# pranavkantgaur/3dscan

Hardware: AMD Instinct MI355X
Metric: Mpixels/s decode+unwrap+triangulate @1920×1080 (higher is better)
Workload: dtype f64

## Files before the change

### 3dscan_amd/csrc/sl3d_capi_context.cpp

```cpp
#include "sl3d_capi_internal.h"

static thread_local std::string g_create_err;

int sl3d_fail(sl3d_ctx *c, int code, const std::string &msg)
{
    if (c) c->err = msg;
    else g_create_err = msg;
    return code;
}

int sl3d_caught(sl3d_ctx *c, std::string *other) noexcept
{
    int code = SL3D_E_INTERNAL;
    const char *what = "unknown C++ exception";
    char buf[256];
    try {
        throw;
    } catch (const std::bad_alloc &) {
        code = SL3D_E_NOMEM;
        what = "out of host memory (std::bad_alloc)";
    } catch (const std::exception &e) {
        snprintf(buf, sizeof buf, "internal error: %s", e.what());
        what = buf;
    } catch (...) {
    }
    try {
        if (other) *other = what;
        else if (c) c->err = what;
        else g_create_err = what;
    } catch (...) {
    }
    return code;
}

extern "C" const char *sl3d_version(void) { return SL3D_VERSION_STRING " (gfx950, hip)"; }

extern "C" const char *sl3d_strerror(int s)
{
    switch (s) {
    case SL3D_OK: return "ok";
    case SL3D_E_INVALID_ARG: return "invalid argument";
    case SL3D_E_NO_DEVICE: return "no HIP device available (this library has no CPU fallback)";
    case SL3D_E_HIP: return "HIP runtime error";
    case SL3D_E_STATE: return "call order violated";
    case SL3D_E_UNSUPPORTED: return "unsupported configuration";
    case SL3D_E_NOMEM: return "out of memory";
    case SL3D_E_INTERNAL: return "internal error (a C++ exception was stopped at the C boundary)";
    default: return "unknown status";
    }
}

extern "C" const char *sl3d_last_error(const sl3d_ctx *ctx) { return ctx ? ctx->err.c_str() : g_create_err.c_str(); }

// ... 116 lines not shown
    x->quad_blocks = mask_prepare_blocks(P);
    CREATE_CHK(hipHostMalloc((void **)&x->h_quad_part, V * (size_t)x->quad_blocks * sizeof(unsigned long long), hipHostMallocMapped));
    memset((void *)x->h_quad_part, 0, V * (size_t)x->quad_blocks * sizeof(unsigned long long));
    CREATE_CHK(hipHostGetDevicePointer((void **)&x->d_quad_part, (void *)x->h_quad_part, 0));
    x->quad_seq.assign(V, 0u);
    x->quad_sum_seq.assign(V, 0u);
    x->quad_sum.assign(V, 0u);
    x->quad_last.assign(V, ~0u);
    x->quad_src.resize(V);
    for (size_t v = 0; v < V; v++) x->quad_src[v] = (int)v;
    x->quad_kind.assign(V, 0);
    x->pend.assign(V, sl3d_ctx::PendingMask());
    x->eager_mask = (c.flags & SL3D_FLAG_EAGER_MASK) != 0;
    if (!x->keep && P.F == 3) {
        x->mi_part_stride = fused_maskin_part_stride(P);
        x->mi_part_words = fused_maskin_part_words(P);
        CREATE_CHK(hipHostMalloc((void **)&x->h_mi_part, V * (size_t)x->mi_part_stride * sizeof(unsigned), hipHostMallocMapped));
        memset((void *)x->h_mi_part, 0, V * (size_t)x->mi_part_stride * sizeof(unsigned));
        CREATE_CHK(hipHostGetDevicePointer((void **)&x->d_mi_part, (void *)x->h_mi_part, 0));
    }
    CREATE_CHK(hipMemsetAsync(x->d_mask, 0, V * P.mask_view_stride, x->stream));
    CREATE_CHK(hipMemsetAsync(x->d_frames, 0, V * P.view_stride, x->stream));
    CREATE_CHK(hipMemsetAsync(x->d_valid, 0, V * P.px_view_stride, x->stream));
    CREATE_CHK(hipMemsetAsync(x->d_points, 0, V * P.px_view_stride * 3 * sizeof(float), x->stream));
    CREATE_CHK(hipMemsetAsync(x->d_band, 0, V * P.px_view_stride, x->stream));
    P.frames = x->d_frames; P.mask = x->d_mask; P.points = x->d_points; P.valid = x->d_valid; P.band = x->d_band;
    {
        static std::mutex mu;
        static std::set<int> verified;
        std::lock_guard<std::mutex> lk(mu);
        if (!verified.count(c.device)) {
            std::vector<float> tab;
            build_atan_tables(tab);
            const size_t n = (size_t)SL3D_ATAN_T1 * SL3D_ATAN_T2;
            float *d_tab = nullptr;
            unsigned *d_cnt = nullptr, h_cnt = 0;
            CREATE_CHK(hipMalloc((void **)&d_tab, 2 * n * sizeof(float)));
            CREATE_CHK(hipMalloc((void **)&d_cnt, sizeof(unsigned)));
            CREATE_CHK(hipMemcpyAsync(d_tab, tab.data(), 2 * n * sizeof(float), hipMemcpyHostToDevice, x->stream));
            CREATE_CHK(hipMemsetAsync(d_cnt, 0, sizeof(unsigned), x->stream));
            CREATE_CHK((hipError_t)launch_atan_selfcheck(d_tab, d_tab + n, d_cnt, x->stream));
            CREATE_CHK(hipMemcpyAsync(&h_cnt, d_cnt, sizeof(unsigned), hipMemcpyDeviceToHost, x->stream));
            CREATE_CHK(hipStreamSynchronize(x->stream));
            (void)hipFree(d_tab);
            (void)hipFree(d_cnt);
            if (h_cnt != 0) {
                g_create_err = "device atan2 differs from the host libm atan2 on " + std::to_string(h_cnt) +
                               " of 521731 lattice points: bit-exact parity cannot be guaranteed on this host/GPU pair";
                        return SL3D_E_UNSUPPORTED;
            }
            verified.insert(c.device);
        }
    }
    if (x->keep) {
        const size_t n = V * P.px_view_stride;
        for (int a = 0; a < 2; a++) {
            ALLOC(P.wrapped[a], n); ALLOC(P.unwrapped[a], n); ALLOC(P.code[a], n);
            ALLOC(P.valid_axis[a], n); ALLOC(P.dbg3[a], n); ALLOC(P.dbg4[a], n);
            CREATE_CHK(hipMemsetAsync(P.wrapped[a], 0, n * 4, x->stream));
            CREATE_CHK(hipMemsetAsync(P.unwrapped[a], 0, n * 4, x->stream));
            CREATE_CHK(hipMemsetAsync(P.code[a], 0xff, n * 4, x->stream));
            CREATE_CHK(hipMemsetAsync(P.valid_axis[a], 0, n, x->stream));
            CREATE_CHK(hipMemsetAsync(P.dbg3[a], 0, n, x->stream));
            CREATE_CHK(hipMemsetAsync(P.dbg4[a], 0, n, x->stream));
        }
        ALLOC(P.cpmap, n * 2); ALLOC(P.ipoints, n * 3);
        CREATE_CHK(hipMemsetAsync(P.cpmap, 0, n * 16, x->stream));
        CREATE_CHK(hipMemsetAsync(P.ipoints, 0, n * 24, x->stream));
    }
#if defined(SL3D_MEASURE) && defined(SL3D_TRACE)
    {
        const size_t blocks = ((((size_t)(P.pitch >> 2) * P.H + 255) / 256) + 7) & ~(size_t)7;
        x->dbg_words = V * blocks * 4 * 8;
        ALLOC(P.dbg, x->dbg_words);
        CREATE_CHK(hipMemsetAsync(P.dbg, 0, x->dbg_words * sizeof(unsigned long long), x->stream));
    }
#endif
    CREATE_CHK(hipStreamSynchronize(x->stream));
#undef ALLOC
#undef CREATE_CHK
    unwind.p = nullptr;
    *out = x;
    return SL3D_OK;
}
SL3D_CATCH(nullptr)

extern "C" void sl3d_destroy(sl3d_ctx *x)
try {
    if (!x) return;
    DeviceGuard dev_guard_(x->cfg.device);
    for (int l = 0; l < 2; l++)
        if (x->lane[l]) (void)hipStreamSynchronize(x->lane[l]);
    if (x->stream) (void)hipStreamSynchronize(x->stream);
    for (int l = 0; l < 2; l++) {
        if (x->ev_lane[l]) (void)hipEventDestroy(x->ev_lane[l]);
        if (x->lane[l]) (void)hipStreamDestroy(x->lane[l]);
    }
    if (x->ev_main) (void)hipEventDestroy(x->ev_main);
    for (void *p : x->allocs) (void)hipFree(p);
    if (x->h_counts) (void)hipHostFree(x->h_counts);
    if (x->h_quad_part) (void)hipHostFree((void *)x->h_quad_part);
    if (x->h_mi_part) (void)hipHostFree((void *)x->h_mi_part);
    for (hipEvent_t e : x->ev_up) (void)hipEventDestroy(e);
    for (hipEvent_t e : x->ev_done) (void)hipEventDestroy(e);
    for (hipEvent_t e : x->ev_down) (void)hipEventDestroy(e);
    if (x->s_h2d) (void)hipStreamDestroy(x->s_h2d);
// ... 160 lines not shown
```

### 3dscan_amd/csrc/sl3d_ctx.h

```cpp
#pragma once
#include <hip/hip_runtime.h>

#include <string>
#include <vector>

#include "../../include/sl3d.h"
#include "sl3d_internal.h"
#include "sl3d_lanes.h"

using namespace sl3d;

struct sl3d_ctx {
    sl3d_config cfg{};
    KParams P{};
    DevCal C{};
    SynthParams S{};
    bool have_cal = false;
    int rig = 0;
    bool keep = false;
    bool own_stream = false;
    hipStream_t stream = nullptr;
    hipEvent_t ev0 = nullptr, ev1 = nullptr;
    bool lanes_ok = false;
    hipStream_t lane[2] = {nullptr, nullptr};
// ... 8 lines not shown
    volatile unsigned long long *h_quad_part = nullptr;
    unsigned long long *d_quad_part = nullptr;
    int quad_blocks = 0;
    std::vector<unsigned> quad_seq;
    std::vector<int> quad_src;
    mutable std::vector<unsigned> quad_sum_seq, quad_sum;
    mutable std::vector<unsigned> quad_last;
    unsigned mask_seq = 0;
    struct PendingMask {
        bool pending = false;
        bool ours = false;
        uintptr_t origin = 0;
        size_t stride = 0;
        int lo = 0, hi = 0;
    };
    std::vector<PendingMask> pend;
    int n_pending = 0;
    bool eager_mask = false;
    volatile unsigned *h_mi_part = nullptr;
    unsigned *d_mi_part = nullptr;
    unsigned mi_part_stride = 0, mi_part_words = 0;
    std::vector<uint8_t> quad_kind;
    struct { int n_views = 0, cmode = 0; bool keep = false, prefer_gated = false, maskin = false; } last_fused;
    float *d_points = nullptr;
    unsigned *d_blk_cnt = nullptr;
    unsigned long long *d_blk_off = nullptr;
    unsigned long long *d_total = nullptr;
    float *d_cloud = nullptr;
    float *d_reg = nullptr;
    uint8_t *d_raw = nullptr;
    bool raw_map_valid = false;
    double Kc_raw[9] = {0}, dc_raw[5] = {0};
    uint8_t *d_und = nullptr;
    size_t und_bytes = 0;
    double und_key[16] = {0};
    bool und_map_valid = false;
    hipStream_t s_h2d = nullptr, s_d2h = nullptr;
    std::vector<hipEvent_t> ev_up, ev_done, ev_down;
    float *d_clouds = nullptr;
    unsigned *d_blk_cnt_all = nullptr;
    unsigned long long *d_blk_off_all = nullptr, *d_totals = nullptr;
    unsigned *d_seg_counts = nullptr;
    unsigned long long *d_seg_offsets = nullptr;
    float *d_packed = nullptr;
    std::vector<uint8_t> scan_state;
    bool clouds_ready = false;
    unsigned long long *h_counts = nullptr;
    uint8_t *d_texture = nullptr;
    uint8_t *d_cloud_rgb = nullptr;
    std::vector<char> have_texture;
    double *d_cam_tab = nullptr;
    size_t cam_tab_doubles = 0;
    float2 *d_proj_disp = nullptr;
    RadEntry *d_proj_rad = nullptr;
    uint8_t *d_pattern = nullptr, *d_profile = nullptr;
    size_t pattern_pitch = 0;
    uint8_t *d_colrow = nullptr;
    size_t colrow_bytes = 0;
    DevCal *d_cal = nullptr;
    size_t mask_rows = 0;
    size_t dbg_words = 0;
};

__attribute__((visibility("hidden"))) int sl3d_fail(sl3d_ctx *c, int code, const std::string &msg);
#define fail sl3d_fail
__attribute__((visibility("hidden"))) int sl3d_caught(sl3d_ctx *c, std::string *err_of_other_owner = nullptr) noexcept;
#define SL3D_CATCH(ctx) catch (...) { return sl3d_caught(ctx); }
#define SL3D_CATCH_RETURN(value) catch (...) { (void)sl3d_caught(nullptr); return value; }
#define SL3D_CATCH_VOID catch (...) { (void)sl3d_caught(nullptr); }
__attribute__((visibility("hidden"))) int sl3d_process_views_enqueue(sl3d_ctx *x, int n_views, const uint8_t *const *planes, size_t stride, float *xyz,
                                                                     size_t xyz_view_stride, uint8_t *valid, size_t valid_view_stride, size_t out_width);
__attribute__((visibility("hidden"))) int sl3d_process_views_wait(sl3d_ctx *x);

#define HIPCHK(c, call)                                                                             \
    do {                                                                                            \
        hipError_t e_ = (call);                                                                     \
        if (e_ != hipSuccess)                                                                       \
            return fail((c), SL3D_E_HIP, std::string(#call) + ": " + hipGetErrorString(e_));        \
    } while (0)

#define HIPCHK_DRAIN(c, call)                                                                       \
    do {                                                                                            \
        hipError_t e_ = (call);                                                                     \
        if (e_ != hipSuccess) {                                                                     \
            (void)hipStreamSynchronize((c)->stream);                                                \
            return fail((c), SL3D_E_HIP, std::string(#call) + ": " + hipGetErrorString(e_));        \
        }                                                                                           \
    } while (0)

struct DeviceGuard {
    int prev = -1, dev;
    hipError_t err = hipSuccess;
    explicit DeviceGuard(int d) : dev(d)
    {
        if (hipGetDevice(&prev) != hipSuccess) prev = -1;
        if (prev != dev) err = hipSetDevice(dev);
    }
    ~DeviceGuard()
    {
        if (prev >= 0 && prev != dev) (void)hipSetDevice(prev);
    }
    DeviceGuard(const DeviceGuard &) = delete;
    DeviceGuard &operator=(const DeviceGuard &) = delete;
};
#define ON_DEVICE_QUIET(x)                 \
    DeviceGuard dev_guard_((x)->cfg.device); \
// ... 10 lines not shown
```

### 3dscan_amd/csrc/sl3d_fused.h

```cpp
#pragma once
#include <stddef.h>
#include <stdlib.h>
#include "sl3d_device.h"
#include "sl3d_maskbits.h"

#define SL3D_BLOCK 256
#define SL3D_OCC 4
#define SL3D_SMALL_BLOCK SL3D_BLOCK

#if !defined(SL3D_MEASURE) || !defined(SL3D_ABLATE)
#undef SL3D_ABLATE
#define SL3D_ABLATE 0
#endif
#if defined(SL3D_MEASURE) && defined(SL3D_TRACE)
#define SL3D_STAMP(k)                                                                                                               \
    do {                                                                                                                            \
           \
        if ((CMODE & 2) == 0 && !KEEP && P.dbg)                                                                                           \
            P.dbg[(((size_t)blockIdx.y * gridDim.x + blockIdx.x) * 4 + (threadIdx.x >> 6)) * 8 + (k)] = wall_clock64();              \
    } while (0)
#else
#define SL3D_STAMP(k)
#endif
#ifdef SL3D_MEASURE
#define SL3D_ABLATE_RT(P) ((P).ablate)
#else
#define SL3D_ABLATE_RT(P) 0
#endif

namespace sl3d {


struct PixelResult {
    float x, y, z;
    bool valid;
};

template <typename CalP>
__device__ __forceinline__ PixelResult parity_chain(const KParams &P, CalP Cp, const PinnedRows &PR, int gx, int gy, double cu, double cv, float wv,
                                                    float wh, int code_v, int code_h, size_t keep_off)
{
    PixelResult R;
    const float nanv = __builtin_nanf("");
    R.x = R.y = R.z = nanv;
    const bool in_v = gx >= 1 && gx <= P.fullW - 2;
    const bool in_h = gy >= 1 && gy <= P.fullH - 2;
    const float uvv = unwrap_value(wv, code_v), uhv = unwrap_value(wh, code_h);
    const float uv = in_v ? uvv : 0.0f;
    const float uh = in_h ? uhv : 0.0f;
    long cx, cy;
    double cxd, cyd;
    const bool okx = correspond(uv, P.fwv, P.PW, cx, cxd);
    const bool oky = correspond(uh, P.fwh, P.PH, cy, cyd);
    R.valid = okx && oky;
    P.wrapped[0][keep_off] = wv;
    P.wrapped[1][keep_off] = wh;
    P.unwrapped[0][keep_off] = uv;
    P.unwrapped[1][keep_off] = uh;
    P.code[0][keep_off] = code_v;
    P.code[1][keep_off] = code_h;
    P.cpmap[2 * keep_off + 0] = R.valid ? cx : 0;
    P.cpmap[2 * keep_off + 1] = R.valid ? cy : 0;
    if (R.valid) {
        double up, vp, X[3];
        const auto &C = *Cp;
        if (C.proj.identity) {
            up = cxd;
            vp = cyd;
        } else {
            undistort_reproject(cxd, cyd, C.proj, up, vp);
        }
        triangulate_px(C, PR, cu, cv, up, vp, X);
        R.x = (float)X[0];
        R.y = (float)X[1];
        R.z = (float)X[2];
        P.ipoints[3 * keep_off + 0] = X[0];
        P.ipoints[3 * keep_off + 1] = X[1];
        P.ipoints[3 * keep_off + 2] = X[2];
    }
    return R;
}

__device__ __forceinline__ bool correspond_px(const KParams &P, int gx, int gy, float wv, float wh, int code_v, int code_h, int &cx, int &cy)
{
    const bool in_v = gx >= 1 && gx <= P.fullW - 2;
    const bool in_h = gy >= 1 && gy <= P.fullH - 2;
    float uvv = unwrap_value(wv, code_v), uhv = unwrap_value(wh, code_h);
    asm volatile("" : "+v"(uvv));
    asm volatile("" : "+v"(uhv));
    float uv = in_v ? uvv : 0.0f;
    float uh = in_h ? uhv : 0.0f;
    asm volatile("" : "+v"(uv));
    asm volatile("" : "+v"(uh));
    long lx, ly;
    double dxd, dyd;
    const bool okx = correspond(uv, P.fwv, P.PW, lx, dxd);
    const bool oky = correspond(uh, P.fwh, P.PH, ly, dyd);
    cx = (int)lx;
    cy = (int)ly;
    return okx && oky;
}

template <int RIG, typename CalP>
__device__ __forceinline__ void triangulate_from(const KParams &P, CalP Cp, const PinnedRows &PR, double cu, double cv, int cx, int cy, float2 d, bool table,
                                                 const RadEntry *s_rad, float &x, float &y, float &z)
{
    const auto &C = *Cp;
    const double cxd = (double)cx, cyd = (double)cy;
    double X[3];
    bool singular = false;
    if (RIG == 3) {
        const double dx = cxd - C.proj.cx, dy = cyd - C.proj.cy;
        const double x0 = dx * C.proj.ifx, y0 = dy * C.proj.ify;
        const double s = radial_lookup(s_rad, P.proj_rad_scale, fma(x0, x0, y0 * y0));
        triangulate_camframe(C, PR, cu, cv, fma(dx, s, cxd), fma(dy, s, cyd), X, singular);
    } else if (RIG == 1) {
        triangulate_camframe(C, PR, cu, cv, cxd, cyd, X, singular);
    } else if (RIG == 2) {
        triangulate_camframe(C, PR, cu, cv, cxd + (double)d.x, cyd + (double)d.y, X, singular);
    } else {
        double up = cxd, vp = cyd;
        if (table) {
            up = cxd + (double)d.x;
            vp = cyd + (double)d.y;
        } else if (!C.proj.identity) {
            undistort_reproject(cxd, cyd, C.proj, up, vp);
        }
        triangulate_px(C, PR, cu, cv, up, vp, X);
    }
    x = (float)X[0];
    y = (float)X[1];
    z = (float)X[2];
    if (RIG != 0 && singular) x = y = z = 0.0f;
}

struct Item {
    unsigned tile;
    int cq, row;
    int gx0, gy;
    int v_begin, v_end;
    bool alive;
    unsigned lane_off;
};

template <bool KIND2 = true>
__device__ __forceinline__ void cam_table_request(const KParams &P, const Item &it, double (&t)[8])
{
    const size_t i0 = (size_t)it.row * P.pitch + (size_t)it.cq * 4;
    if (!KIND2 || P.use_cam_table == 1) {
        const double2 *tp = (const double2 *)(P.cam_tab + i0);
        const double2 a = tp[0], b = tp[1];
        t[0] = a.x; t[1] = a.y; t[2] = b.x; t[3] = b.y;
    } else {
        const double2 *tp = (const double2 *)(P.cam_tab + 2 * i0);
        const double2 a = tp[0], b = tp[1], c = tp[2], d = tp[3];
// ... 282 lines not shown
            if (PLANES == 1 || i < N) {
                g[a][i] = ldg32(vb + (size_t)(pg + (unsigned)i * psv), lo);
                iv[a][i] = ldg32(vb + (size_t)(pg + (unsigned)(N + i) * psv), lo);
            }
        }
    }
}

template <int NMAX, int PLANES>
__device__ __forceinline__ void decode_gray(const unsigned (&g)[2][NMAX], const unsigned (&iv)[2][NMAX], int Nv, int Nh, unsigned (&code)[2][2])
{
#pragma unroll
    for (int a = 0; a < 2; a++) {
        const int N = a == 0 ? Nv : Nh;
        const unsigned H = 0x80808080u;
        unsigned bacc = 0;
        unsigned hi = 0, lo = 0;
        if (PLANES >= 2) {
            int pad = NMAX - N;
            if (PLANES == 3) pad = __builtin_amdgcn_readfirstlane(pad);
            asm volatile("" : "+s"(pad));
#pragma unroll
            for (int i = 0; i < NMAX; i++) {
                const unsigned x = g[a][i], y = iv[a][i];
                const unsigned t = (x | H) - (y & ~H);
                const unsigned ge = __builtin_amdgcn_bitop3_b32(x, y, t, 0xB2);
                const unsigned Hm = i >= pad ? H : 0u;
                bacc = __builtin_amdgcn_bitop3_b32(bacc, ge, Hm, 0x78);
                if (i < NMAX - 8) hi = (hi << 1) | (bacc >> 7);
                else lo = (lo << 1) | (bacc >> 7);
            }
            code[a][0] = __builtin_amdgcn_perm(hi, lo, 0x05010400u);
            code[a][1] = __builtin_amdgcn_perm(hi, lo, 0x07030602u);
            continue;
        }
#pragma unroll
        for (int i = 0; i < NMAX; i++) {
            if (i < N) {
                const unsigned x = g[a][i], y = iv[a][i];
                const unsigned t = (x | H) - (y & ~H);
                const unsigned ge = __builtin_amdgcn_bitop3_b32(x, y, t, 0xB2);
                bacc = __builtin_amdgcn_bitop3_b32(bacc, ge, H, 0x78);
                if (i < N - 8) hi = (hi << 1) | (bacc >> 7);
                else lo = (lo << 1) | (bacc >> 7);
            }
        }
        code[a][0] = __builtin_amdgcn_perm(hi, lo, 0x05010400u);
        code[a][1] = __builtin_amdgcn_perm(hi, lo, 0x07030602u);
    }
}

template <bool RCP_TAB>
__device__ __forceinline__ unsigned pixel_A(const KParams &P, const Item &it, int F, int i, int k, unsigned vbits, const unsigned (&f)[2][4],
                                            const unsigned (&code)[2][2], const double *s_rcp, int *pair_cp)
{
    const int sh = 8 * i;
    const int code_v = (int)((code[0][0] >> (16 * i)) & 0xffffu);
    const int code_h = (int)((code[1][0] >> (16 * i)) & 0xffffu);
    const AtanK AK = atan_consts<true>();
    float wv = wrapped_phase<RCP_TAB>(F, (f[0][0] >> sh) & 255, (f[0][1] >> sh) & 255, (f[0][2] >> sh) & 255, (f[0][3] >> sh) & 255, s_rcp, AK);
    float wh = wrapped_phase<RCP_TAB>(F, (f[1][0] >> sh) & 255, (f[1][1] >> sh) & 255, (f[1][2] >> sh) & 255, (f[1][3] >> sh) & 255, s_rcp, AK);
    wv = shift_pi(wv);
    wh = shift_pi(wh);
    int cx, cy;
    const bool ok = correspond_px(P, it.gx0 + k, it.gy, wv, wh, code_v, code_h, cx, cy) && ((vbits >> i) & 1u);
    pair_cp[3 * i] = ok ? cx : 0;
    pair_cp[3 * i + 1] = ok ? cy : 0;
    return ok ? 1u : 0u;
}

template <bool RCP_TAB>
__device__ __forceinline__ void phase_A_pair(const KParams &P, const Item &it, int F, int j, unsigned &vbits, unsigned (&f)[2][4], unsigned (&code)[2][2],
                                             const double *s_rcp, int *pair_cp, unsigned &vout)
{
    const unsigned ok0 = pixel_A<RCP_TAB>(P, it, F, 0, 2 * j, vbits, f, code, s_rcp, pair_cp), ok1 = pixel_A<RCP_TAB>(P, it, F, 1, 2 * j + 1, vbits, f, code, s_rcp, pair_cp);
    vout = (vout >> 16) | (ok0 << 16) | (ok1 << 24);
#pragma unroll
    for (int a = 0; a < 2; a++) {
#pragma unroll
        for (int p = 0; p < 4; p++) f[a][p] >>= 16;
        code[a][0] = code[a][1];
    }
    vbits >>= 2;
}

template <bool RCP_TAB, bool UNROLL>
__device__ __forceinline__ unsigned phase_A(const KParams &P, const Item &it, int F, unsigned vbits, unsigned (&f)[2][4], unsigned (&code)[2][2],
                                            const double *s_rcp, int *my_cp)
{
    unsigned vout = 0;
#pragma unroll(UNROLL ? 2 : 1)
    for (int j = 0; j < 2; j++) {
        int j8 = j * 8;
        if (!UNROLL) asm volatile("" : "+v"(j8));
        phase_A_pair<RCP_TAB>(P, it, F, j, vbits, f, code, s_rcp, my_cp + (UNROLL ? 6 * j : ((j8 << 1) + j8) >> 2), vout);
    }
    return vout;
}

template <bool RCP_TAB>
__device__ __forceinline__ void wrapped_quad(int F, const unsigned (&f)[2][4], const double *s_rcp, float (&w)[2][4])
{
    const AtanK AK = atan_consts<true>();
#pragma unroll
    for (int k = 0; k < 4; k++) {
        const int sh = 8 * k;
#pragma unroll
        for (int a = 0; a < 2; a++)
            w[a][k] = shift_pi(wrapped_phase<RCP_TAB>(F, (f[a][0] >> sh) & 255, (f[a][1] >> sh) & 255, (f[a][2] >> sh) & 255, (f[a][3] >> sh) & 255, s_rcp, AK));
    }
}

__device__ __forceinline__ unsigned correspond_quad(const KParams &P, const Item &it, unsigned vbits, const float (&w)[2][4], const unsigned (&code)[2][2], int *my_cp)
{
    unsigned vout = 0;
#pragma unroll
    for (int k = 0; k < 4; k++) {
        const int code_v = (int)((code[0][k >> 1] >> (16 * (k & 1))) & 0xffffu);
        const int code_h = (int)((code[1][k >> 1] >> (16 * (k & 1))) & 0xffffu);
        int cx, cy;
        const bool ok = correspond_px(P, it.gx0 + k, it.gy, w[0][k], w[1][k], code_v, code_h, cx, cy) && ((vbits >> k) & 1u);
        my_cp[3 * k] = ok ? cx : 0;
        my_cp[3 * k + 1] = ok ? cy : 0;
        vout |= (ok ? 1u : 0u) << (8 * k);
    }
    return vout;
}

__device__ __forceinline__ void gather_B(const KParams &P, bool proj_table, const int *my_cp, float2 (&d)[4])
{
#pragma unroll
    for (int k = 0; k < 4; k++) d[k] = make_float2(0.f, 0.f);
    if (proj_table) {
        const GLOBAL_AS uint8_t *tab = opaque((const uint8_t *)P.proj_disp);
        const unsigned pw = (unsigned)P.PW;
#pragma unroll
        for (int k = 0; k < 4; k++) d[k] = ldg_f2(tab, ((unsigned)my_cp[3 * k + 1] * pw + (unsigned)my_cp[3 * k]) * 8u);
    }
}

template <int RIG, bool UNROLL>
__device__ __forceinline__ void phase_B(const KParams &P, const DevCal *Cglobal, const PinnedRows &PR, bool proj_table, unsigned vout, float2 (&d)[4],
                                        const double *my_cam, const int *my_cp, float *my_xyz, const RadEntry *s_rad)
{
    const float nanv = __builtin_nanf("");
    unsigned vb = vout;
#pragma unroll(UNROLL ? 2 : 1)
    for (int j = 0; j < 2; j++) {
        int j8 = j * 8;
        if (!UNROLL) asm volatile("" : "+v"(j8));
        const int pair_words = UNROLL ? 6 * j : ((j8 << 1) + j8) >> 2;
        const int *cp = my_cp + pair_words;
        float *xyz = my_xyz + pair_words;
        const double *cam = my_cam + (UNROLL ? 4 * j : j8 >> 1);
#pragma unroll
        for (int i = 0; i < 2; i++) {
            float x, y, z;
            triangulate_from<RIG>(P, opaque_const(Cglobal), PR, cam[2 * i], cam[2 * i + 1], cp[3 * i], cp[3 * i + 1], d[i], proj_table, s_rad, x, y, z);
            const bool ok = ((vb >> (8 * i)) & 1u) != 0u;
            xyz[3 * i + 0] = ok ? x : nanv;
            xyz[3 * i + 1] = ok ? y : nanv;
            xyz[3 * i + 2] = ok ? z : nanv;
        }
        d[0] = d[2];
        d[1] = d[3];
        vb >>= 16;
    }
}

template <bool RCP_TAB>
__device__ __forceinline__ unsigned parity_pixels(const KParams &P, const DevCal *Cglobal, const PinnedRows &PR, const Item &it, int F, unsigned vbits,
                                                  const unsigned (&f)[2][4], const unsigned (&code)[2][2], const double *s_rcp, const double *my_cam,
                                                  float *my_xyz, size_t px)
{
// ... 109 lines not shown
            if ((vout >> (8 * k)) & 1u) {
                wbase[3 * rank + 0] = q[3 * k + 0];
                wbase[3 * rank + 1] = q[3 * k + 1];
                wbase[3 * rank + 2] = q[3 * k + 2];
                rank++;
            }
    }
    wave_lds_handoff();
    const unsigned chunks = (3u * total + 3u) >> 2;
    typedef float f32x4 __attribute__((ext_vector_type(4)));
    const f32x4 *wb4 = (const f32x4 *)wbase;
    GLOBAL_AS uint8_t *out = opaque_out(slot);
#pragma unroll
    for (int c3 = 0; c3 < 3; c3++) {
        const unsigned i = (unsigned)c3 * 64u + lane_;
        if (i < chunks) stg_nt(out, lane_ * 16u + (unsigned)c3 * 1024u, wb4[i]);
    }
    wave_lds_handoff();
}

template <bool KEEP, bool FGEN, bool SEG>
__device__ __forceinline__ unsigned valid_bits(const Item &it, int F, const MaskQuad &m)
{
    if (SEG && !it.alive) return 0u;
    return (FGEN && F == 5) ? 0u : (!KEEP && (SL3D_ABLATE & 2)) ? 0xfu : mask_quad_bits(m);
}

template <int RIG>
struct RadialLds {
    __device__ __forceinline__ static RadEntry *get() { return nullptr; }
};
template <>
struct RadialLds<3> {
    __device__ __forceinline__ static RadEntry *get()
    {
        __shared__ RadEntry tab[SL3D_RAD_NODES];
        return tab;
    }
};

template <bool KEEP, int NMAX, bool FGEN, bool EXACT, int RIG, int CMODE, bool RCPT, bool EARLY_>
__global__ __launch_bounds__(RCPT ? SL3D_BLOCK : SL3D_SMALL_BLOCK, SL3D_OCC) void k_fused(const KParams P, const DevCal *__restrict__ Cglobal, int first_view, int n_views, int vpt)
{
    constexpr bool SEG = (CMODE & 2) != 0;
    constexpr bool MASKIN = (CMODE & 4) != 0;
    constexpr int BLK = RCPT ? SL3D_BLOCK : SL3D_SMALL_BLOCK;
    static_assert((CMODE & ~6) == 0, "0 = dense planes, 2 = segmented clouds (1 was round 2's look-back compaction), + 4 = MASKIN");
    static_assert(!MASKIN || (!KEEP && RIG != 0 && (RCPT ? !EARLY_ : EARLY_)),
                  "MASKIN: the pipelined small-launch instantiations, and the gated large-launch ones (views known to be sparsely selected)");
    static_assert(!(KEEP && CMODE != 0), "the parity mode writes dense planes");
    static_assert(!(KEEP && RIG != 0), "the parity mode evaluates everything with the reference's operation order");
    __shared__ __attribute__((aligned(16))) float s_xyz[BLK * 12];
    __shared__ __attribute__((aligned(16))) double s_cam[BLK * 8];
    __shared__ __attribute__((aligned(16))) double s_rcp[RCPT ? SL3D_RCP_TAB : 1];
    RadEntry *const s_rad = RadialLds<RIG>::get();
    static_assert(RIG != 3 || SL3D_BLOCK == SL3D_RAD_NODES, "one table node per thread");
    SL3D_STAMP(0);
    constexpr bool PIPE = !KEEP && RIG != 0;
    static_assert(RCPT || EARLY_ == PIPE, "the small-launch instantiation: early requests iff pipelined");
    constexpr bool EARLY = EARLY_ && PIPE;
    constexpr bool REQ_FIRST = PIPE;
    typedef unsigned u32x4 __attribute__((ext_vector_type(4)));
    u32x4 rad_node = {0u, 0u, 0u, 0u};
    if (RIG == 3) rad_node = ((const u32x4 *)P.proj_rad)[(blockIdx.x & 7u) * SL3D_RAD_STRIDE + threadIdx.x];
    if (!REQ_FIRST) {
        if (RIG == 3) ((u32x4 *)s_rad)[threadIdx.x] = rad_node;
        if (RCPT) fill_rcp_table(s_rcp);
        if (RCPT || RIG == 3) __syncthreads();
    }
    SL3D_STAMP(1);
    const int F = FGEN ? P.F : 3;
    float *my_xyz = s_xyz + threadIdx.x * 12;
    double *my_cam = s_cam + threadIdx.x * 8;
    int *my_cp = (int *)my_xyz;
    constexpr bool UNROLL = !RCPT;
#ifdef SL3D_NO_SPLIT
    constexpr bool SPLIT = false;
#else
    constexpr bool SPLIT = EARLY;
#endif

    constexpr int PLANES = EXACT ? 1 : (!KEEP && NMAX <= 12) ? ((MASKIN && RCPT) ? 3 : 2) : 0;
    const int Nv = EXACT ? NMAX : P.Nv, Nh = EXACT ? NMAX : P.Nh;
    const bool proj_table = RIG == 2 || (RIG == 0 && !KEEP && P.proj_disp != nullptr);

    Item it;
    MaskQuad mq;
    double camt[8] = {0, 0, 0, 0, 0, 0, 0, 0};
    unsigned mbits = 0u;
    mrow_t mw0 = {0u, 0u}, mw1 = mw0, mw2 = mw0, mw3 = mw0, mw4 = mw0;
    bool mfast = false;
    unsigned f[2][4], g[2][NMAX], iv[2][NMAX], code[2][2];
    if (!item_begin<RIG, SEG, REQ_FIRST, BLK, MASKIN>(P, Cglobal, blockIdx.x, (int)blockIdx.y, first_view, n_views, vpt, it, mq, camt, my_cam, mw0, mw1, mw2, mw3, mw4, mfast)) return;
    if (MASKIN) it.v_end = it.v_begin + 1;
    if (REQ_FIRST) {
        if (EARLY) {
            issue_fringe<FGEN>(P, it.v_begin, it.lane_off, F, Nv, f);
            issue_gray<NMAX, PLANES>(P, it.v_begin, it.lane_off, F, Nv, Nh, g, iv);
        }
        if (RCPT) fill_rcp_table(s_rcp);
        if (RIG == 3) ((u32x4 *)s_rad)[threadIdx.x] = rad_node;
        if (RCPT || RIG == 3) __syncthreads();
        if (!SEG && !it.alive) return;
        if (MASKIN) {
            if (it.alive) mbits = maskin_finish(P, it, it.v_begin, it.v_begin - first_view, mw0, mw1, mw2, mw3, mw4, mfast);
            maskin_count(P, it, it.v_begin, mbits);
        }
        if (P.use_cam_table) cam_table_finish<RIG, !MASKIN>(P, Cglobal, it, camt, my_cam);
    }
    SL3D_STAMP(2);
    unsigned vb_next = 0;
    if (PIPE) {
        vb_next = MASKIN ? (mbits & 0xfu) : valid_bits<KEEP, FGEN, SEG>(it, F, mq);
        if (!MASKIN && it.v_begin + 1 < it.v_end) mq = load_mask_quad(P, it.v_begin + 1, it.lane_off);
        if (!EARLY && vb_next != 0) {
            issue_fringe<FGEN>(P, it.v_begin, it.lane_off, F, Nv, f);
            issue_gray<NMAX, PLANES>(P, it.v_begin, it.lane_off, F, Nv, Nh, g, iv);
        }
    }
    const PinnedRows PR = pinned_rows<RIG>(Cglobal);
    constexpr bool DEFER = PIPE;
    unsigned pvout = 0;
    auto store_view = [&](int v, unsigned vo) {
        const size_t p = (size_t)v * P.px_view_stride + (size_t)it.lane_off;
        if (MASKIN && it.alive) maskin_store(P, it, v, mbits);
        if (SEG) store_segment(P, it, v, vo, s_xyz, my_xyz);
        else store_quad<KEEP>(P, s_xyz, my_xyz, p, vo);
    };
    for (int view = it.v_begin; view < it.v_end; view++) {
        unsigned vbits;
        if (PIPE) {
            vbits = vb_next;
        } else {
            vbits = valid_bits<KEEP, FGEN, SEG>(it, F, mq);
            if (view + 1 < it.v_end) mq = load_mask_quad(P, view + 1, it.lane_off);
        }
        const size_t px = (size_t)view * P.px_view_stride + (size_t)it.lane_off;
        unsigned vout = 0;
        if (KEEP) parity_init(P, px, vbits);
        if (!DEFER && !SEG && (KEEP || vbits == 0)) fill_nan(my_xyz);
        if (!PIPE && vbits != 0) {
            issue_fringe<FGEN>(P, view, it.lane_off, F, Nv, f);
            issue_gray<NMAX, PLANES>(P, view, it.lane_off, F, Nv, Nh, g, iv);
        }
        if (view == it.v_begin) SL3D_STAMP(3);
        float w[2][4];
        if (SPLIT && vbits != 0) {
            wrapped_quad<RCPT>(F, f, s_rcp, w);
            __builtin_amdgcn_sched_barrier(0);
        }
        if (vbits != 0) decode_gray<NMAX, PLANES>(g, iv, Nv, Nh, code);
        if (view == it.v_begin) SL3D_STAMP(4);
        unsigned vb_pre = 0;
        if (PIPE) {
            vb_pre = MASKIN ? 0u : valid_bits<KEEP, FGEN, SEG>(it, F, mq);
            asm volatile("" : "+v"(vb_pre));
        }
        if (DEFER) {
            if (view > it.v_begin) store_view(view - 1, pvout);
            if (!SEG && vbits == 0) fill_nan(my_xyz);
        }
        if (vbits != 0) {
            if (KEEP) vout = parity_pixels<RCPT>(P, Cglobal, PR, it, F, vbits, f, code, s_rcp, my_cam, my_xyz, px);
            else if (SPLIT) vout = correspond_quad(P, it, vbits, w, code, my_cp);
            else vout = phase_A<RCPT, UNROLL>(P, it, F, vbits, f, code, s_rcp, my_cp);
        }
        if (view == it.v_begin) SL3D_STAMP(5);
        if (PIPE && view + 1 < it.v_end) {
            vb_next = vb_pre;
            if (!MASKIN) mq = load_mask_quad(P, min(view + 2, it.v_end - 1), it.lane_off);
            if (vb_next != 0) {
                issue_fringe<FGEN>(P, view + 1, it.lane_off, F, Nv, f);
                issue_gray<NMAX, PLANES>(P, view + 1, it.lane_off, F, Nv, Nh, g, iv);
            }
        }
        if (!KEEP && vbits != 0) {
            float2 d[4];
            gather_B(P, proj_table, my_cp, d);
            phase_B<RIG, UNROLL>(P, Cglobal, PR, proj_table, vout, d, my_cam, my_cp, my_xyz, s_rad);
        }
        if (DEFER) {
            if (view == it.v_begin) SL3D_STAMP(6);
            pvout = vout;
            continue;
        }
        if (SEG) {
            store_segment(P, it, view, vout, s_xyz, my_xyz);
            continue;
        }
        if (view == it.v_begin) SL3D_STAMP(6);
        store_quad<KEEP>(P, s_xyz, my_xyz, px, vout);
        if (view == it.v_begin) SL3D_STAMP(7);
    }
    if (DEFER) {
        store_view(it.v_end - 1, pvout);
        SL3D_STAMP(7);
    }
}

struct FusedChoice {
    int nmax;
    bool exact, small;
    bool early;
};
inline FusedChoice choose_fused(bool keep, bool fgen, int cmode, int nv, int nh, int n_views, bool prefer_gated, int rig)
{
    FusedChoice c;
    const int m = nv > nh ? nv : nh;
    c.exact = !keep && !fgen && nv == nh && nv >= 6 && nv <= 12;
    if (c.exact) c.nmax = nv;
    else if (!keep && m <= 12 && nv > 0 && nh > 0) c.nmax = m < 6 ? 6 : m;
    else if (!keep) c.nmax = SL3D_MAX_GRAY;
    else c.nmax = m <= 8 ? 8 : (m <= 12 ? 12 : SL3D_MAX_GRAY);
    c.small = !keep && !fgen && n_views <= SL3D_SMALL_LAUNCH_VIEWS && !prefer_gated;
#ifdef SL3D_MEASURE
    if (getenv("SL3D_NO_SMALL")) c.small = false;
#endif
    const bool pipelined = !keep && rig != 0 && m <= 12 && nv > 0 && nh > 0;
// ... 112 lines not shown
```

### 3dscan_amd/csrc/sl3d_internal.h

```cpp
#pragma once
#include <stddef.h>
#include <stdint.h>

#include <hip/hip_vector_types.h>

#define SL3D_MASK_HALO 2
#define SL3D_MASK_LPAD 16
#define SL3D_ATAN_T1 511
#define SL3D_ATAN_T2 1021
#define SL3D_MAX_GRAY 16
#define SL3D_SEG_POINTS 256
#define SL3D_SMALL_LAUNCH_VIEWS 4

namespace sl3d {

struct Intr {
    double K[9];
    double ifx, ify, cx, cy;
    double k1, k2, p1, p2, k3;
    int has_dist;
    int affine;
    int has_tan;
    int plain;
    int identity;
// ... 37 lines not shown
    uintptr_t origin[SL3D_SMALL_LAUNCH_VIEWS];
    size_t stride;
    int bx0, bx1, r0, r1;
    int lo, hi;
    unsigned *part;
    unsigned part_stride;
    unsigned seq;
};

struct KParams {
    int W, H;
    int fullW, fullH;
    int col0, row0;
    int PW, PH;
    int F, Nv, Nh;
    int fwv, fwh;
    int ncodes_v, ncodes_h;
    int ablate;
    int pitch;
    int planes_per_view;
    size_t plane_stride;
    size_t view_stride;
    int mpitch;
    size_t mask_view_stride;
    const uint8_t *frames;
    const uint8_t *mask;
    const uint8_t *band;
    const float2 *proj_disp;
    const RadEntry *proj_rad;
    float proj_rad_scale;
    const double *cam_tab;
    int cam_tab_kind;
    int use_cam_table;
    float *points;
    uint8_t *valid;
    size_t px_view_stride;
    float *clouds;
    unsigned long long *cloud_totals;
    int n_tiles;
    int prefer_gated;
    unsigned *seg_counts;
    unsigned long long *seg_offsets;
    int n_segs;
    unsigned long long *dbg;
    float *wrapped[2];
    float *unwrapped[2];
    int32_t *code[2];
    uint8_t *valid_axis[2];
    uint8_t *dbg3[2];
    uint8_t *dbg4[2];
    int64_t *cpmap;
    double *ipoints;
    MaskIn mi;
};
static_assert(SL3D_SMALL_LAUNCH_VIEWS == 4, "KParams::mi_origin holds one entry per view of a small launch");

int launch_fused(const KParams &P, const DevCal *d_cal, int rig, int first_view, int n_views, bool keep, int cmode, void *stream, bool prefer_gated = false,
                 const MaskIn *mi = nullptr);
int fused_kernel_name(const KParams &P, int rig, int n_views, bool keep, int cmode, char *buf, size_t cap, bool prefer_gated = false, bool maskin = false);
bool fused_maskin_available(const KParams &P, int rig, int n_views, bool keep);
unsigned fused_maskin_part_stride(const KParams &P);
unsigned fused_maskin_part_words(const KParams &P);
int launch_seg_scan(const KParams &P, int first_view, int n_views, void *stream);
int launch_seg_close(const KParams &P, int first_view, int n_views, float *dst, size_t dst_view_stride_points, void *stream);
int launch_seg_close_scan(const KParams &P, int first_view, int n_views, float *dst, size_t dst_view_stride_points, unsigned long long capacity_points,
                          void *stream);
int launch_seg_register(const KParams &P, int view, float *out, const float R4[4], float tx, float ty, float tz, void *stream);
int fused_tiles(const KParams &P);
int launch_mask_prepare(const KParams &P, int first_view, int n_views, const MaskSrc &S, unsigned long long *partials, unsigned seq, void *stream);
int mask_prepare_blocks(const KParams &P);
int launch_to_colrow(const KParams &P, int view, int which, void *dst, void *stream);
int launch_mask_from_colrow(const KParams &P, const int *sel, int gx0, int gy0, int ncols, int nrows, uint8_t *raw, void *stream);
int launch_proj_table(const DevCal *d_cal, int PW, int PH, float2 *out, void *stream);
int launch_radial_table(const DevCal *d_cal, int which, double r2max, RadEntry *out, void *stream);
int launch_cam_table(const KParams &P, const DevCal *d_cal, int kind, double *out, void *stream);
int launch_wrap(const KParams &P, int view, int axis, void *stream);
int launch_unwrap(const KParams &P, int view, int axis, void *stream);
int launch_corr(const KParams &P, int view, void *stream);
int launch_tri(const KParams &P, const DevCal &C, int view, void *stream);
int launch_compact(const KParams &P, int view, unsigned *block_counts, unsigned long long *block_offsets, unsigned long long *total,
                   float *cloud, const uint8_t *texture, uint8_t *rgb_out, void *stream);
int launch_compact_views(const KParams &P, int first_view, int n_views, unsigned *block_counts, unsigned long long *block_offsets,
                         unsigned long long *totals, float *clouds, void *stream);
int launch_register(const float *in, float *out, long n, const float R4[4], float tx, float ty, float tz, void *stream);
int launch_synth(const KParams &P, const DevCal &C, const SynthParams &S, int view, void *stream);
int launch_undistort(const uint8_t *src, size_t sstride, uint8_t *dst, size_t dstride, int width, int height, int cn, const double K[9],
                     const double dist[5], short *m1, unsigned short *m2, bool build_map, void *stream);
int launch_undistort_planes(const uint8_t *src, size_t spitch, size_t splane, uint8_t *dst, size_t dpitch, size_t dplane, int width, int height,
                            int n_planes, const double K[9], const double dist[5], short *m1, unsigned short *m2, bool build_map, void *stream);
int launch_pattern(uint8_t *dst, size_t pitch, int PW, int PH, int axis, const uint8_t *profile, void *stream);
int launch_atan_selfcheck(const float *tab_phi, const float *tab_shift, unsigned *mismatches, void *stream);

}
```

Baseline: 95140.

## Replace per-pixel atan2 phase with lattice-separator table correspondence decode

```diff
diff --git a/3dscan_amd/csrc/sl3d_capi_context.cpp b/3dscan_amd/csrc/sl3d_capi_context.cpp
--- a/3dscan_amd/csrc/sl3d_capi_context.cpp
+++ b/3dscan_amd/csrc/sl3d_capi_context.cpp
@@ -1,4 +1,5 @@
 #include "sl3d_capi_internal.h"
+#include "sl3d_corr.h"
 
 static thread_local std::string g_create_err;
 
@@ -221,6 +222,28 @@
             verified.insert(c.device);
         }
     }
+    if (!x->keep) {
+        static std::mutex mu;
+        static cr_dir *dirs = nullptr;
+        static int ndirs = 0;
+        {
+            std::lock_guard<std::mutex> lk(mu);
+            if (!dirs) dirs = cr_sorted_lattice(&ndirs);
+        }
+        const int Lv = std::min(P.PW, (int)std::min<long>((long)P.fwv << std::min(P.Nv, 16), 1L << 30));
+        const int Lh = std::min(P.PH, (int)std::min<long>((long)P.fwh << std::min(P.Nh, 16), 1L << 30));
+        std::vector<uint32_t> tab(((size_t)Lv + Lh + 2 + 1023) & ~(size_t)1023, 0u);
+        if (dirs && Lv > 0 && Lh > 0 && cr_build_table(dirs, ndirs, P.fwv, P.Nv, P.PW, tab.data()) == Lv &&
+            cr_build_table(dirs, ndirs, P.fwh, P.Nh, P.PH, tab.data() + Lv + 1) == Lh) {
+            ALLOC(x->d_sep, tab.size());
+            CREATE_CHK(hipMemcpyAsync(x->d_sep, tab.data(), tab.size() * sizeof(uint32_t), hipMemcpyHostToDevice, x->stream));
+            P.sep = x->d_sep;
+            P.sep_l[0] = Lv;
+            P.sep_l[1] = Lh;
+            cr_consts(P.fwv, &P.sep_a[0], &P.sep_b[0]);
+            cr_consts(P.fwh, &P.sep_a[1], &P.sep_b[1]);
+        }
+    }
     if (x->keep) {
         const size_t n = V * P.px_view_stride;
         for (int a = 0; a < 2; a++) {
diff --git a/3dscan_amd/csrc/sl3d_corr.h b/3dscan_amd/csrc/sl3d_corr.h
--- /dev/null
+++ b/3dscan_amd/csrc/sl3d_corr.h
@@ -0,0 +1,112 @@
+#pragma once
+#include <math.h>
+#include <stdint.h>
+#include <stdlib.h>
+
+#ifdef __HIPCC__
+#define SL3D_CR_FN __host__ __device__ __forceinline__
+#else
+#define SL3D_CR_FN static inline
+#endif
+
+#ifndef PI_REF
+#define PI_REF 22.0 / 7.0
+#endif
+
+#define SL3D_CR_FW_MAX 64
+#define SL3D_CR_EST_ERR 0.005
+#define SL3D_CR_SEP_TOL 0.05
+#define SL3D_CR_T1 255
+#define SL3D_CR_T2 510
+
+static inline double cr_chain(float phi, int code, int fw)
+{
+    const float w = (float)((double)phi + PI_REF);
+    const float u = (float)((double)w + code * 2.0 * PI_REF);
+    return rint((double)fw * ((double)u / (2.0 * PI_REF)));
+}
+
+SL3D_CR_FN float cr_ytil(float r, int swap, int neg2, int neg1, float A, float B)
+{
+    const float at = r * fmaf(-0.273f, r, 1.0584f);
+    float q = swap ? 1.57079637f - at : at;
+    q = neg2 ? 3.14159274f - q : q;
+    return fmaf(A, neg1 ? -q : q, B);
+}
+SL3D_CR_FN int cr_jt(float ytil, int fw)
+{
+    const int j = (int)ytil;
+    return j < 1 ? 1 : (j > fw ? fw : j);
+}
+SL3D_CR_FN void cr_consts(int fw, float *A, float *B)
+{
+    *A = (float)((double)fw * 7.0 / 44.0);
+    *B = (float)((double)fw * 0.5 + 1.0);
+}
+
+SL3D_CR_FN uint32_t cr_pack(int s1, int s2) { return (uint32_t)(uint16_t)(int16_t)s2 | ((uint32_t)(uint16_t)(int16_t)(-s1) << 16); }
+SL3D_CR_FN int cr_reach(uint32_t e, int t1, int t2)
+{
+    const int s2 = (int)(int16_t)(e & 0xffffu), ns1 = (int)(int16_t)(e >> 16);
+    return s2 * t1 + ns1 * t2 >= 0;
+}
+SL3D_CR_FN int cr_decide(const uint32_t *tab, int L, int fw, int code, int jt, int t1, int t2)
+{
+    const int idx = fw * code + jt;
+    return idx - (cr_reach(tab[idx < L ? idx : L], t1, t2) ? 0 : 1);
+}
+
+typedef struct {
+    int16_t t1, t2;
+    float phi;
+} cr_dir;
+
+static inline int cr_half(int t1, int t2) { return t1 < 0 ? 0 : ((t1 > 0 || t2 > 0) ? 1 : 2); }
+static inline int cr_dir_cmp(const void *pa, const void *pb)
+{
+    const cr_dir *a = (const cr_dir *)pa, *b = (const cr_dir *)pb;
+    const int ha = cr_half(a->t1, a->t2), hb = cr_half(b->t1, b->t2);
+    if (ha != hb) return ha < hb ? -1 : 1;
+    const long c = (long)a->t2 * b->t1 - (long)a->t1 * b->t2;
+    return c > 0 ? -1 : (c < 0 ? 1 : 0);
+}
+
+static inline cr_dir *cr_sorted_lattice(int *n)
+{
+    cr_dir *d = (cr_dir *)malloc(sizeof(cr_dir) * (2 * SL3D_CR_T1 + 1) * (2 * SL3D_CR_T2 + 1));
+    int k = 0;
+    if (!d) return NULL;
+    for (int t1 = -SL3D_CR_T1; t1 <= SL3D_CR_T1; t1++)
+        for (int t2 = -SL3D_CR_T2; t2 <= SL3D_CR_T2; t2++) {
+            if (t1 == 0 && t2 == 0) continue;
+            d[k].t1 = (int16_t)t1;
+            d[k].t2 = (int16_t)t2;
+            d[k].phi = (float)atan2((double)t1, (double)t2);
+            k++;
+        }
+    qsort(d, (size_t)k, sizeof(cr_dir), cr_dir_cmp);
+    *n = k;
+    return d;
+}
+
+static inline int cr_build_table(const cr_dir *d, int n, int fw, int N, int limit, uint32_t *out)
+{
+    if (fw < 2 || fw > SL3D_CR_FW_MAX || N < 0 || N > 16 || limit < 1) return -1;
+    const long span = (long)fw << N;
+    const int L = (int)(span < limit ? span : limit);
+    out[0] = 0;
+    for (int X = 1; X <= L; X++) {
+        const int c = (X - 1) / fw, j = X - fw * c;
+        int lo = 0, hi = n;
+        while (lo < hi) {
+            const int m = lo + (hi - lo) / 2;
+            if (cr_chain(d[m].phi, c, fw) >= (double)X) hi = m;
+            else lo = m + 1;
+        }
+        if (lo == 0 || lo == n) return -1;
+        const double ideal = (j - 0.5) * (44.0 / 7.0) / fw - 22.0 / 7.0;
+        if (fabs(atan2((double)d[lo].t1, (double)d[lo].t2) - ideal) > SL3D_CR_SEP_TOL) return -1;
+        out[X] = cr_pack(d[lo].t1, d[lo].t2);
+    }
+    return L;
+}
diff --git a/3dscan_amd/csrc/sl3d_ctx.h b/3dscan_amd/csrc/sl3d_ctx.h
--- a/3dscan_amd/csrc/sl3d_ctx.h
+++ b/3dscan_amd/csrc/sl3d_ctx.h
@@ -84,6 +84,7 @@
     double *d_cam_tab = nullptr;
     size_t cam_tab_doubles = 0;
     float2 *d_proj_disp = nullptr;
+    uint32_t *d_sep = nullptr;
     RadEntry *d_proj_rad = nullptr;
     uint8_t *d_pattern = nullptr, *d_profile = nullptr;
     size_t pattern_pitch = 0;
diff --git a/3dscan_amd/csrc/sl3d_fused.h b/3dscan_amd/csrc/sl3d_fused.h
--- a/3dscan_amd/csrc/sl3d_fused.h
+++ b/3dscan_amd/csrc/sl3d_fused.h
@@ -3,6 +3,7 @@
 #include <stdlib.h>
 #include "sl3d_device.h"
 #include "sl3d_maskbits.h"
+#include "sl3d_corr.h"
 
 #define SL3D_BLOCK 256
 #define SL3D_OCC 4
@@ -101,6 +102,34 @@
     return okx && oky;
 }
 
+__device__ __forceinline__ int corr_estimate(unsigned a, unsigned b, unsigned c, unsigned d, float A, float B, int fw)
+{
+    const unsigned ay = __builtin_amdgcn_sad_u16(a, b, 0u), ax = __builtin_amdgcn_sad_u16(c, d, 0u);
+    const unsigned lo = min(ay, ax), hi = max(max(ay, ax), 1u);
+    const float r = (float)lo * __builtin_amdgcn_rcpf((float)hi);
+    return cr_jt(cr_ytil(r, ay > ax, c < d, a < b, A, B), fw);
+}
+__device__ __forceinline__ int corr_decide(const uint32_t *tab, int L, int fw, int code, int jt, unsigned a, unsigned b, unsigned c, unsigned d)
+{
+    const int t1 = (int)a - (int)b;
+    int t2 = (int)c - (int)d;
+    t2 += (t1 | t2) == 0 ? 1 : 0;
+    return cr_decide(tab, L, fw, code, jt, t1, t2);
+}
+__device__ __forceinline__ bool correspond_sep_px(const KParams &P, int gx, int gy, int xv, int xh, int &cx, int &cy)
+{
+    const bool in_v = gx >= 1 && gx <= P.fullW - 2;
+    const bool in_h = gy >= 1 && gy <= P.fullH - 2;
+    cx = in_v ? xv : 0;
+    cy = in_h ? xh : 0;
+    return cx <= P.PW - 1 && cy <= P.PH - 1;
+}
+__device__ __forceinline__ void lattice_args(int F, unsigned i0, unsigned i1, unsigned i2, unsigned i3, unsigned &a, unsigned &b, unsigned &c, unsigned &d)
+{
+    if (F == 3) { a = i0; b = i2; c = 2u * i1; d = i0 + i2; }
+    else { a = i3; b = i1; c = i0; d = i2; }
+}
+
 template <int RIG, typename CalP>
 __device__ __forceinline__ void triangulate_from(const KParams &P, CalP Cp, const PinnedRows &PR, double cu, double cv, int cx, int cy, float2 d, bool table,
                                                  const RadEntry *s_rad, float &x, float &y, float &z)
@@ -489,11 +518,27 @@
 
 template <bool RCP_TAB>
 __device__ __forceinline__ unsigned pixel_A(const KParams &P, const Item &it, int F, int i, int k, unsigned vbits, const unsigned (&f)[2][4],
-                                            const unsigned (&code)[2][2], const double *s_rcp, int *pair_cp)
+                                            const unsigned (&code)[2][2], const double *s_rcp, const uint32_t *s_sep, int *pair_cp)
 {
     const int sh = 8 * i;
     const int code_v = (int)((code[0][0] >> (16 * i)) & 0xffffu);
     const int code_h = (int)((code[1][0] >> (16 * i)) & 0xffffu);
+    if (s_sep) {
+        int X[2];
+#pragma unroll
+        for (int ax = 0; ax < 2; ax++) {
+            unsigned a, b, c, d;
+            lattice_args(F, (f[ax][0] >> sh) & 255, (f[ax][1] >> sh) & 255, (f[ax][2] >> sh) & 255, (f[ax][3] >> sh) & 255, a, b, c, d);
+            const int fw = ax ? P.fwh : P.fwv;
+            const int jt = corr_estimate(a, b, c, d, P.sep_a[ax], P.sep_b[ax], fw);
+            X[ax] = corr_decide(s_sep + (ax ? P.sep_l[0] + 1 : 0), P.sep_l[ax], fw, ax ? code_h : code_v, jt, a, b, c, d);
+        }
+        int cx, cy;
+        const bool ok = correspond_sep_px(P, it.gx0 + k, it.gy, X[0], X[1], cx, cy) && ((vbits >> i) & 1u);
+        pair_cp[3 * i] = ok ? cx : 0;
+        pair_cp[3 * i + 1] = ok ? cy : 0;
+        return ok ? 1u : 0u;
+    }
     const AtanK AK = atan_consts<true>();
     float wv = wrapped_phase<RCP_TAB>(F, (f[0][0] >> sh) & 255, (f[0][1] >> sh) & 255, (f[0][2] >> sh) & 255, (f[0][3] >> sh) & 255, s_rcp, AK);
     float wh = wrapped_phase<RCP_TAB>(F, (f[1][0] >> sh) & 255, (f[1][1] >> sh) & 255, (f[1][2] >> sh) & 255, (f[1][3] >> sh) & 255, s_rcp, AK);
@@ -508,9 +553,10 @@
 
 template <bool RCP_TAB>
 __device__ __forceinline__ void phase_A_pair(const KParams &P, const Item &it, int F, int j, unsigned &vbits, unsigned (&f)[2][4], unsigned (&code)[2][2],
-                                             const double *s_rcp, int *pair_cp, unsigned &vout)
-{
-    const unsigned ok0 = pixel_A<RCP_TAB>(P, it, F, 0, 2 * j, vbits, f, code, s_rcp, pair_cp), ok1 = pixel_A<RCP_TAB>(P, it, F, 1, 2 * j + 1, vbits, f, code, s_rcp, pair_cp);
+                                             const double *s_rcp, const uint32_t *s_sep, int *pair_cp, unsigned &vout)
+{
+    const unsigned ok0 = pixel_A<RCP_TAB>(P, it, F, 0, 2 * j, vbits, f, code, s_rcp, s_sep, pair_cp),
+                   ok1 = pixel_A<RCP_TAB>(P, it, F, 1, 2 * j + 1, vbits, f, code, s_rcp, s_sep, pair_cp);
     vout = (vout >> 16) | (ok0 << 16) | (ok1 << 24);
 #pragma unroll
     for (int a = 0; a < 2; a++) {
@@ -523,21 +569,37 @@
 
 template <bool RCP_TAB, bool UNROLL>
 __device__ __forceinline__ unsigned phase_A(const KParams &P, const Item &it, int F, unsigned vbits, unsigned (&f)[2][4], unsigned (&code)[2][2],
-                                            const double *s_rcp, int *my_cp)
+                                            const double *s_rcp, const uint32_t *s_sep, int *my_cp)
 {
     unsigned vout = 0;
 #pragma unroll(UNROLL ? 2 : 1)
     for (int j = 0; j < 2; j++) {
         int j8 = j * 8;
         if (!UNROLL) asm volatile("" : "+v"(j8));
-        phase_A_pair<RCP_TAB>(P, it, F, j, vbits, f, code, s_rcp, my_cp + (UNROLL ? 6 * j : ((j8 << 1) + j8) >> 2), vout);
+        phase_A_pair<RCP_TAB>(P, it, F, j, vbits, f, code, s_rcp, s_sep, my_cp + (UNROLL ? 6 * j : ((j8 << 1) + j8) >> 2), vout);
     }
     return vout;
 }
 
 template <bool RCP_TAB>
-__device__ __forceinline__ void wrapped_quad(int F, const unsigned (&f)[2][4], const double *s_rcp, float (&w)[2][4])
-{
+__device__ __forceinline__ void wrapped_quad(const KParams &P, int F, const unsigned (&f)[2][4], const double *s_rcp, const uint32_t *s_sep, float (&w)[2][4])
+{
+    if (s_sep) {
+        unsigned jq[2] = {0u, 0u};
+#pragma unroll
+        for (int k = 0; k < 4; k++) {
+            const int sh = 8 * k;
+#pragma unroll
+            for (int a = 0; a < 2; a++) {
+                unsigned ta, tb, tc, td;
+                lattice_args(F, (f[a][0] >> sh) & 255, (f[a][1] >> sh) & 255, (f[a][2] >> sh) & 255, (f[a][3] >> sh) & 255, ta, tb, tc, td);
+                jq[a] |= (unsigned)corr_estimate(ta, tb, tc, td, P.sep_a[a], P.sep_b[a], a ? P.fwh : P.fwv) << sh;
+            }
+        }
+        w[0][0] = __uint_as_float(jq[0]);
+        w[1][0] = __uint_as_float(jq[1]);
+        return;
+    }
     const AtanK AK = atan_consts<true>();
 #pragma unroll
     for (int k = 0; k < 4; k++) {
@@ -548,7 +610,8 @@
     }
 }
 
-__device__ __forceinline__ unsigned correspond_quad(const KParams &P, const Item &it, unsigned vbits, const float (&w)[2][4], const unsigned (&code)[2][2], int *my_cp)
+__device__ __forceinline__ unsigned correspond_quad(const KParams &P, const Item &it, int F, unsigned vbits, const unsigned (&f)[2][4], const float (&w)[2][4],
+                                                    const unsigned (&code)[2][2], const uint32_t *s_sep, int *my_cp)
 {
     unsigned vout = 0;
 #pragma unroll
@@ -556,7 +619,22 @@
         const int code_v = (int)((code[0][k >> 1] >> (16 * (k & 1))) & 0xffffu);
         const int code_h = (int)((code[1][k >> 1] >> (16 * (k & 1))) & 0xffffu);
         int cx, cy;
-        const bool ok = correspond_px(P, it.gx0 + k, it.gy, w[0][k], w[1][k], code_v, code_h, cx, cy) && ((vbits >> k) & 1u);
+        bool ok;
+        if (s_sep) {
+            const int sh = 8 * k;
+            int X[2];
+#pragma unroll
+            for (int a = 0; a < 2; a++) {
+                unsigned ta, tb, tc, td;
+                lattice_args(F, (f[a][0] >> sh) & 255, (f[a][1] >> sh) & 255, (f[a][2] >> sh) & 255, (f[a][3] >> sh) & 255, ta, tb, tc, td);
+                const int jt = (int)((__float_as_uint(w[a][0]) >> sh) & 255u);
+                X[a] = corr_decide(s_sep + (a ? P.sep_l[0] + 1 : 0), P.sep_l[a], a ? P.fwh : P.fwv, a ? code_h : code_v, jt, ta, tb, tc, td);
+            }
+            ok = correspond_sep_px(P, it.gx0 + k, it.gy, X[0], X[1], cx, cy);
+        } else {
+            ok = correspond_px(P, it.gx0 + k, it.gy, w[0][k], w[1][k], code_v, code_h, cx, cy);
+        }
+        ok = ok && ((vbits >> k) & 1u);
         my_cp[3 * k] = ok ? cx : 0;
         my_cp[3 * k + 1] = ok ? cy : 0;
         vout |= (ok ? 1u : 0u) << (8 * k);
@@ -772,7 +850,13 @@
     static_assert(!(KEEP && RIG != 0), "the parity mode evaluates everything with the reference's operation order");
     __shared__ __attribute__((aligned(16))) float s_xyz[BLK * 12];
     __shared__ __attribute__((aligned(16))) double s_cam[BLK * 8];
-    __shared__ __attribute__((aligned(16))) double s_rcp[RCPT ? SL3D_RCP_TAB : 1];
+    constexpr int TABW = KEEP ? 2 * SL3D_RCP_TAB : !RCPT ? 2 : (RIG == 3 ? 2048 : 3072);
+    static_assert(TABW >= 2 * SL3D_RCP_TAB || !RCPT, "the table area holds the reciprocal table too");
+    __shared__ __attribute__((aligned(16))) uint32_t s_tab[TABW];
+    double *const s_rcp = (double *)s_tab;
+    const int sep_words = P.sep_l[0] + P.sep_l[1] + 2;
+    const bool use_sep = !KEEP && RCPT && P.sep != nullptr && sep_words <= TABW;
+    const uint32_t *const s_sep = use_sep ? s_tab : nullptr;
     RadEntry *const s_rad = RadialLds<RIG>::get();
     static_assert(RIG != 3 || SL3D_BLOCK == SL3D_RAD_NODES, "one table node per thread");
     SL3D_STAMP(0);
@@ -783,9 +867,24 @@
     typedef unsigned u32x4 __attribute__((ext_vector_type(4)));
     u32x4 rad_node = {0u, 0u, 0u, 0u};
     if (RIG == 3) rad_node = ((const u32x4 *)P.proj_rad)[(blockIdx.x & 7u) * SL3D_RAD_STRIDE + threadIdx.x];
+    constexpr int SEPQ = (TABW + 4 * BLK - 1) / (4 * BLK);
+    u32x4 sep_q[SEPQ];
+#pragma unroll
+    for (int q = 0; q < SEPQ; q++) {
+        sep_q[q] = u32x4{0u, 0u, 0u, 0u};
+        if (use_sep && q * 4 * BLK < sep_words) sep_q[q] = ((const u32x4 *)P.sep)[q * BLK + threadIdx.x];
+    }
+    auto fill_sep = [&]() {
+        if (use_sep) {
+#pragma unroll
+            for (int q = 0; q < SEPQ; q++)
+                if (q * 4 * BLK < sep_words && (q * BLK + (int)threadIdx.x) * 4 < TABW) ((u32x4 *)s_tab)[q * BLK + threadIdx.x] = sep_q[q];
+        }
+    };
     if (!REQ_FIRST) {
         if (RIG == 3) ((u32x4 *)s_rad)[threadIdx.x] = rad_node;
-        if (RCPT) fill_rcp_table(s_rcp);
+        fill_sep();
+        if (RCPT && !use_sep) fill_rcp_table(s_rcp);
         if (RCPT || RIG == 3) __syncthreads();
     }
     SL3D_STAMP(1);
@@ -814,11 +913,12 @@
     if (!item_begin<RIG, SEG, REQ_FIRST, BLK, MASKIN>(P, Cglobal, blockIdx.x, (int)blockIdx.y, first_view, n_views, vpt, it, mq, camt, my_cam, mw0, mw1, mw2, mw3, mw4, mfast)) return;
     if (MASKIN) it.v_end = it.v_begin + 1;
     if (REQ_FIRST) {
+        fill_sep();
         if (EARLY) {
             issue_fringe<FGEN>(P, it.v_begin, it.lane_off, F, Nv, f);
             issue_gray<NMAX, PLANES>(P, it.v_begin, it.lane_off, F, Nv, Nh, g, iv);
         }
-        if (RCPT) fill_rcp_table(s_rcp);
+        if (RCPT && !use_sep) fill_rcp_table(s_rcp);
         if (RIG == 3) ((u32x4 *)s_rad)[threadIdx.x] = rad_node;
         if (RCPT || RIG == 3) __syncthreads();
         if (!SEG && !it.alive) return;
@@ -866,7 +966,7 @@
         if (view == it.v_begin) SL3D_STAMP(3);
         float w[2][4];
         if (SPLIT && vbits != 0) {
-            wrapped_quad<RCPT>(F, f, s_rcp, w);
+            wrapped_quad<RCPT>(P, F, f, s_rcp, s_sep, w);
             __builtin_amdgcn_sched_barrier(0);
         }
         if (vbits != 0) decode_gray<NMAX, PLANES>(g, iv, Nv, Nh, code);
@@ -882,8 +982,8 @@
         }
         if (vbits != 0) {
             if (KEEP) vout = parity_pixels<RCPT>(P, Cglobal, PR, it, F, vbits, f, code, s_rcp, my_cam, my_xyz, px);
-            else if (SPLIT) vout = correspond_quad(P, it, vbits, w, code, my_cp);
-            else vout = phase_A<RCPT, UNROLL>(P, it, F, vbits, f, code, s_rcp, my_cp);
+            else if (SPLIT) vout = correspond_quad(P, it, F, vbits, f, w, code, s_sep, my_cp);
+            else vout = phase_A<RCPT, UNROLL>(P, it, F, vbits, f, code, s_rcp, s_sep, my_cp);
         }
         if (view == it.v_begin) SL3D_STAMP(5);
         if (PIPE && view + 1 < it.v_end) {
diff --git a/3dscan_amd/csrc/sl3d_internal.h b/3dscan_amd/csrc/sl3d_internal.h
--- a/3dscan_amd/csrc/sl3d_internal.h
+++ b/3dscan_amd/csrc/sl3d_internal.h
@@ -113,6 +113,9 @@
     int64_t *cpmap;
     double *ipoints;
     MaskIn mi;
+    const uint32_t *sep;
+    int sep_l[2];
+    float sep_a[2], sep_b[2];
 };
 static_assert(SL3D_SMALL_LAUNCH_VIEWS == 4, "KParams::mi_origin holds one entry per view of a small launch");
 
```

Result: no change. 94780 (median of 6 runs) (-0.4%).
